# hliuson/ogbench

Measured on AMD Instinct MI355X. Metric: env steps/sec at N=65536 parallel envs, pointmaze-large, 1/2/4/8 MI355X, higher is better.
Workload: dtype f64; 1 GPU; pointmaze-large-navigate-v0; total_envs=65536, num_envs_per_gpu=65536, auto_reset=True, task_id=i%5+1, seed=0, parallelism=env-shard x1 (contiguous blocks, global env_base)

## Files before the change

ogbench_amd/csrc/locomaze.hip:

```cpp
#include <cmath>
#include <cstdlib>
#include <cstring>
#include <deque>
#include <string>
#include <type_traits>
#include <vector>

#include "common.h"
#include "goal_threshold.h"
#include "point_physics.h"
#include "point_contact.h"


namespace ogbx {

constexpr int kMaxCells = 256;
constexpr int kMaxTasks = 8;

struct MazeParams {
  PointModel pm;
  int32_t H, W, num_tasks, loco_type;
  int32_t success_pre, terminate_at_goal, add_noise_to_goal, reward_task_id;
  int32_t max_steps, n_tp_in, n_tp_out, pad_;
  int64_t env_base;
  double goal_tol, tp_radius;
  double tp_in[2][2];
  double tp_out[3][2];
  int32_t tasks[kMaxTasks][4];
  uint8_t wall[kMaxCells];
  uint16_t nbmask[kMaxCells];
};

struct MazeState {
  double* qpos;
  double* goal;
  int32_t* elapsed;
  int32_t* task;
  uint32_t* episode;
};

struct MazeStepConsts {
  const uint16_t* nbmask;
  int64_t env_base;
  double goal_tol;
  double goal_s2max;
  int32_t H, W, max_steps, n_tp_in;
  int32_t success_pre, terminate_at_goal, reward_task_id, add_noise_to_goal;
};

}

struct ogbx_maze_env {
  int32_t device = 0;
  int64_t n = 0;
  ogbx::MazeParams P;
  ogbx::MazeState S{};
  ogbx::MazeParams* Pd = nullptr;
  ogbx::MazeStepConsts C{};
  int16_t* bfs = nullptr;
  uint64_t seed = 0;
  bool was_reset = false;
  double* body_qpos = nullptr;
  double* body_qvel = nullptr;
  int epw = 64;
  int lds_pad = 0;
  bool bound = false;
  double* b_obs = nullptr;
  float* b_reward = nullptr;
  uint8_t *b_term = nullptr, *b_trunc = nullptr, *b_succ = nullptr;
  double* b_final = nullptr;
  int32_t b_auto = 0;
};

namespace ogbx {


#define OGBX_POINT_MODEL(pm, P) constexpr PointModel pm = kPointModel

__device__ inline void stage_wall(const MazeParams& P, uint8_t* wall_s) {
  for (int t = threadIdx.x; t < P.H * P.W; t += blockDim.x) wall_s[t] = P.wall[t];
  __syncthreads();
}

__device__ inline void stage_nbmask(const MazeParams& P, uint16_t* nb_s) {
  for (int t = threadIdx.x; t < P.H * P.W; t += blockDim.x) nb_s[t] = P.nbmask[t];
  __syncthreads();
}

static_assert(kMaxCells == kStepBlock, "one wall-mask entry per thread of a step block");

__device__ __forceinline__ uint16_t nbmask_fetch(const MazeParams* Pp) { return Pp->nbmask[threadIdx.x]; }

__device__ __forceinline__ void nbmask_commit(uint16_t* nb_s, uint16_t v) {
  nb_s[threadIdx.x] = v;
  __syncthreads();
}

__device__ inline bool goal_reached(double x, double y, double gx, double gy, double tol) {
  double dx = x - gx, dy = y - gy;
  return sqrt(fma(dy, dy, dx * dx)) <= tol;
}

__device__ inline bool goal_within(double x, double y, double gx, double gy, double s2max) {
  double dx = x - gx, dy = y - gy;
  return fma(dy, dy, dx * dx) <= s2max;
}

__device__ inline void reset_draws(uint64_t i, uint32_t ep, uint32_t k0, uint32_t k1,
                                   double r[4]) {
  u32x4 a = philox4x32_10({(uint32_t)i, ep, 0u, (uint32_t)(i >> 32)}, k0, k1);
  u32x4 b = philox4x32_10({(uint32_t)i, ep, 1u, (uint32_t)(i >> 32)}, k0, k1);
  r[0] = -1.0 + 2.0 * u01_from(a.x, a.y);
  r[1] = -1.0 + 2.0 * u01_from(a.z, a.w);
  r[2] = -1.0 + 2.0 * u01_from(b.x, b.y);
  r[3] = -1.0 + 2.0 * u01_from(b.z, b.w);
}

__device__ inline int32_t draw_task(const MazeParams& P, uint64_t i, uint32_t ep, uint32_t k0,
                                    uint32_t k1) {
  u32x4 c = philox4x32_10({(uint32_t)i, ep, 2u, (uint32_t)(i >> 32)}, k0, k1);
  return 1 + (int32_t)bounded_u32(c.x, (uint32_t)P.num_tasks);
}

__device__ inline void task_centres(const PointModel& pm, const int32_t* t, double c[4]) {
  c[0] = t[1] * pm.unit - pm.off_x;
  c[1] = t[0] * pm.unit - pm.off_y;
  c[2] = t[3] * pm.unit - pm.off_x;
  c[3] = t[2] * pm.unit - pm.off_y;
}

__device__ inline void reset_noise(const PointModel& pm, const double c[4], int32_t add_noise_to_goal,
                                   const double r[4], double& x, double& y, double& gx, double& gy) {
  x = c[0] + r[0] * pm.unit / 4.0;
  y = c[1] + r[1] * pm.unit / 4.0;
  if (add_noise_to_goal) {
    gx = c[2] + r[2] * pm.unit / 4.0;
    gy = c[3] + r[3] * pm.unit / 4.0;
  } else {
    gx = c[2];
    gy = c[3];
  }
}

__device__ inline void reset_one(const MazeParams& P, int32_t task, const double* task_xy,
                                 const double r[4], double& x, double& y, double& gx,
                                 double& gy) {
  double c[4];
  if (task_xy != nullptr) {
    for (int k = 0; k < 4; ++k) c[k] = task_xy[k];
  } else {
    task_centres(P.pm, P.tasks[task - 1], c);
  }
  reset_noise(P.pm, c, P.add_noise_to_goal, r, x, y, gx, gy);
}

__device__ inline void reset_from_task(const PointModel& pm, const int32_t* t, int32_t add_noise_to_goal,
                                       const double r[4], double& x, double& y, double& gx, double& gy) {
  double c[4];
  task_centres(pm, t, c);
  reset_noise(pm, c, add_noise_to_goal, r, x, y, gx, gy);
}


constexpr int kEpwReplicate = 0x100;

__device__ inline int64_t env_of_lane(int epw, bool* writer) {
  const int lane = threadIdx.x & 63;
  const int e = epw & 0xFF;
  const int64_t wave = ((int64_t)blockIdx.x * kStepBlock + threadIdx.x) >> 6;
  *writer = lane < e;
  if (lane >= e && !(epw & kEpwReplicate)) return -1;
  return wave * e + (lane & (e - 1));
}

__global__ void __launch_bounds__(256) maze_reset_kernel(const MazeParams* __restrict__ Pp, MazeState S, int64_t n,
                                                         const int32_t* task_id,
                                                         const double* task_xy,
                                                         const uint8_t* mask, const double* noise,
                                                         double* obs, double* goal_out,
                                                         uint32_t k0, uint32_t k1) {
  const MazeParams& P = *Pp;
  const PointModel pm = P.pm;
  int64_t i = (int64_t)blockIdx.x * blockDim.x + threadIdx.x;
  if (i >= n) return;
  if (mask != nullptr && mask[i] == 0) return;
  uint32_t ep = S.episode[i] + 1u;
  const uint64_t gi = (uint64_t)(i + P.env_base);
  int32_t task;
  if (P.reward_task_id > 0) task = P.reward_task_id;
  else if (task_id != nullptr) task = task_id[i];
  else task = draw_task(P, gi, ep, k0, k1);
  if (task < 1 || task > P.num_tasks) task = 1;
  double r[4];
  if (noise != nullptr) {
    r[0] = noise[4 * i + 0];
    r[1] = noise[4 * i + 1];
    r[2] = noise[4 * i + 2];
    r[3] = noise[4 * i + 3];
  } else {
    reset_draws(gi, ep, k0, k1, r);
  }
  double x, y, gx, gy;
  reset_one(P, task, task_xy ? task_xy + 4 * i : nullptr, r, x, y, gx, gy);
  S.qpos[2 * i] = x;
  S.qpos[2 * i + 1] = y;
  S.goal[2 * i] = gx;
  S.goal[2 * i + 1] = gy;
  S.elapsed[i] = 0;
  S.task[i] = task;
  S.episode[i] = ep;
  obs[2 * i] = x;
  obs[2 * i + 1] = y;
  goal_out[2 * i] = gx;
  goal_out[2 * i + 1] = gy;
}

#ifdef OGBX_WAVE_STAMPS
__device__ unsigned long long g_wave_stamps[4096 * 4];
#endif

typedef double f64x2 __attribute__((ext_vector_type(2)));

constexpr int64_t kPlainMaxEnvs = (int64_t)1 << 27;

template <bool k32, class T>
__device__ __forceinline__ T* env_elem(T* base, int64_t i) {
  if constexpr (k32) {
    using B = std::conditional_t<std::is_const_v<T>, const char, char>;
    return reinterpret_cast<T*>(reinterpret_cast<B*>(base) + (uint32_t)i * (uint32_t)sizeof(T));
  } else {
    return base + i;
  }
}

template <bool kF64, bool kUntilDone, bool kPlain = false>
__global__ void __launch_bounds__(256) maze_step_kernel(
    const MazeStepConsts C, MazeState S, const void* __restrict__ action_v, int64_t n,
    double* __restrict__ obs, float* __restrict__ reward, uint8_t* __restrict__ terminated,
    uint8_t* __restrict__ truncated, uint8_t* __restrict__ success, int32_t auto_reset, int32_t k_steps_arg,
    double* __restrict__ final_obs, uint32_t k0, uint32_t k1, int epw,
    const MazeParams* __restrict__ Pp, int32_t* __restrict__ steps_taken) {
  static_assert(!(kPlain && kUntilDone), "the plain instantiation is the single auto-reset step");
  const MazeParams& P = *Pp;
  OGBX_POINT_MODEL(pm, P);
  const int32_t k_steps = kPlain ? 1 : k_steps_arg;
  const int32_t n_tp_in = kPlain ? 0 : C.n_tp_in;
  __shared__ uint16_t nb_s[kMaxCells];
#ifdef OGBX_WAVE_STAMPS
  const unsigned long long ws_t0 = wall_clock64(), ws_c0 = clock64();
#endif
#ifdef OGBX_STAGE_STAMPS
  const unsigned long long ps_t0 = __builtin_amdgcn_s_memtime();
  __builtin_amdgcn_sched_barrier(0);
#endif
  bool writer = true;
  int64_t i;
  bool live;
  if constexpr (kPlain) {
    const uint32_t t = blockIdx.x * kStepBlock + threadIdx.x;
    i = t;
    live = t < (uint32_t)n;
  } else {
    i = env_of_lane(epw, &writer);
    live = i >= 0 && i < n;
  }
  asm volatile("" ::"s"(C.H), "s"(C.W), "s"(C.max_steps), "s"(C.goal_tol), "s"(action_v), "s"(S.episode),
               "s"(k_steps_arg));
  double2 q = make_double2(0.0, 0.0), g = q, a0d = q;
  float2 a0f = make_float2(0.0f, 0.0f);
  int32_t el = 0, task = 1;
  uint32_t ep = 0;
  if (live) {
    q = *env_elem<kPlain>(reinterpret_cast<const double2*>(S.qpos), i);
    if (kF64) a0d = *env_elem<kPlain>(reinterpret_cast<const double2*>(action_v), i);
    else a0f = *env_elem<kPlain>(reinterpret_cast<const float2*>(action_v), i);
    g = *env_elem<kPlain>(reinterpret_cast<const double2*>(S.goal), i);
    el = *env_elem<kPlain>(static_cast<const int32_t*>(S.elapsed), i);
  }
  const uint16_t nbv = C.nbmask[threadIdx.x];
#ifdef OGBX_STAGE_STAMPS
  asm volatile("s_waitcnt vmcnt(0)" ::: "memory");
  OGBX_PS_AT(1);
  path_stamp_store(0, ps_t0);
#endif
  nbmask_commit(nb_s, nbv);
  OGBX_PS_AT(2);
  if (!live) return;
  bool have_te = k_steps > 1 || n_tp_in > 0 || el + 1 >= C.max_steps;
  {
    const double ddx = q.x - g.x, ddy = q.y - g.y, lim = C.goal_tol + 2.0;
    have_te |= ddx * ddx + ddy * ddy <= lim * lim;
  }
  if (have_te) {
    ep = *env_elem<kPlain>(static_cast<const uint32_t*>(S.episode), i);
    task = *env_elem<kPlain>(static_cast<const int32_t*>(S.task), i);
  }
  const uint64_t gi = (uint64_t)(i + C.env_base);
  double x = q.x, y = q.y, gx = g.x, gy = g.y;
  bool reset_any = false;
  bool done = false;
  int32_t taken = 0;
  double dx_ = x, dy_ = y;
  int32_t del_ = el;

  for (int32_t k = 0; k < k_steps; ++k) {
    if (kUntilDone) {
      if (__all(done)) break;
    }
    const int64_t o = kPlain ? i : (int64_t)k * n + i;
    double dx, dy;
    if (kF64) {
      const double2 a = k == 0 ? a0d : reinterpret_cast<const double2*>(action_v)[o];
      dx = 0.2 * a.x;
      dy = 0.2 * a.y;
    } else {
      const float2 a = k == 0 ? a0f : reinterpret_cast<const float2*>(action_v)[o];
      dx = (double)(0.2f * a.x);
      dy = (double)(0.2f * a.y);
    }
    bool succ = false;
    if (C.success_pre) succ = goal_within(x, y, gx, gy, C.goal_s2max);
    x = x + dx;
    y = y + dy;
    if constexpr (kPlain) {
#pragma unroll 1
      for (int32_t rep = 0; rep < k_steps_arg; ++rep) point_step_as(pm, nb_s, C.H, C.W, &x, &y);
    } else {
      point_step_as(pm, nb_s, C.H, C.W, &x, &y);
    }
    if (!C.success_pre) succ = goal_within(x, y, gx, gy, C.goal_s2max);
    const double ox = x, oy = y;
    if (n_tp_in > 0) {
      for (int t = 0; t < n_tp_in; ++t) {
        if (goal_reached(x, y, P.tp_in[t][0], P.tp_in[t][1], P.tp_radius * 1.5)) {
          u32x4 c = philox4x32_10({(uint32_t)gi, ep, 0x100u + (uint32_t)el, (uint32_t)(gi >> 32)},
                                  k0 ^ kTagMazeTeleport, k1);
          int o_idx = (int)bounded_u32(c.x, (uint32_t)P.n_tp_out);
          x = P.tp_out[o_idx][0];
          y = P.tp_out[o_idx][1];
          break;
        }
      }
    }
    float rew = succ ? 1.0f : 0.0f;
    if (C.reward_task_id > 0) rew -= 1.0f;
    const bool term = succ && C.terminate_at_goal;
    el += 1;
    const bool trunc = el >= C.max_steps;
    const bool write = writer && (!kUntilDone || !done);
    if (write) {
      __builtin_nontemporal_store(rew, env_elem<kPlain>(reward, o));
      __builtin_nontemporal_store((uint8_t)term, env_elem<kPlain>(terminated, o));
      __builtin_nontemporal_store((uint8_t)trunc, env_elem<kPlain>(truncated, o));
      __builtin_nontemporal_store((uint8_t)succ, env_elem<kPlain>(success, o));
    }
    OGBX_PS_AT(8);
    double wx = ox, wy = oy;
    if (auto_reset && (term || trunc)) {
      if (!have_te) {
        ep = *env_elem<kPlain>(static_cast<const uint32_t*>(S.episode), i);
        task = *env_elem<kPlain>(static_cast<const int32_t*>(S.task), i);
        have_te = true;
      }
      if (final_obs != nullptr && writer)
        *env_elem<kPlain>(reinterpret_cast<double2*>(final_obs), o) = make_double2(ox, oy);
      ep += 1u;
      reset_any = true;
      double r[4];
      reset_draws(gi, ep, k0, k1, r);
      reset_from_task(pm, P.tasks[task - 1], C.add_noise_to_goal, r, x, y, gx, gy);
      el = 0;
      wx = x;
      wy = y;
    }
    if (write) __builtin_nontemporal_store(f64x2{wx, wy}, env_elem<kPlain>(reinterpret_cast<f64x2*>(obs), o));
    if (kUntilDone && !done) {
      taken = k + 1;
      done = term || trunc;
      dx_ = x;
      dy_ = y;
      del_ = el;
    }
  }
  if (kUntilDone) {
    x = dx_;
    y = dy_;
    el = del_;
    if (writer) steps_taken[i] = taken;
  }
  if (!writer) return;
  OGBX_PS_AT(9);
  __builtin_nontemporal_store(f64x2{x, y}, env_elem<kPlain>(reinterpret_cast<f64x2*>(S.qpos), i));
  __builtin_nontemporal_store(el, env_elem<kPlain>(S.elapsed, i));
  if (reset_any) {
    *env_elem<kPlain>(reinterpret_cast<double2*>(S.goal), i) = make_double2(gx, gy);
    *env_elem<kPlain>(S.episode, i) = ep;
  }
  OGBX_PS_AT(10);
#ifdef OGBX_WAVE_STAMPS
  {
    const unsigned long long t1 = wall_clock64(), c1 = clock64();
    const int64_t w = ((int64_t)blockIdx.x * kStepBlock + threadIdx.x) >> 6;
    if ((threadIdx.x & 63) == 0 && w < 4096) {
      g_wave_stamps[4 * w + 0] = ws_t0;
      g_wave_stamps[4 * w + 1] = t1;
      g_wave_stamps[4 * w + 2] = c1 - ws_c0;
    }
  }
#endif
}

template <bool kF64>
__global__ void __launch_bounds__(256) point_physics_kernel(const MazeParams* __restrict__ Pp,
                                                            const double* qpos_in,
                                                            const void* action_v, int64_t n,
                                                            double* qpos_out,
                                                            uint8_t* contact_out, int epw) {
  OGBX_POINT_MODEL(pm, (*Pp));
  __shared__ uint16_t nb_s[kMaxCells];
  bool writer;
  const int64_t i = env_of_lane(epw, &writer);
  const bool live = i >= 0 && i < n;
  const uint16_t nbv = nbmask_fetch(Pp);
  double x = 0.0, y = 0.0, ax = 0.0, ay = 0.0;
  if (live) {
    x = qpos_in[2 * i];
    y = qpos_in[2 * i + 1];
    if (kF64) {
      const double* a = (const double*)action_v;
      ax = 0.2 * a[2 * i];
      ay = 0.2 * a[2 * i + 1];
    } else {
      const float* a = (const float*)action_v;
      ax = (double)(0.2f * a[2 * i]);
      ay = (double)(0.2f * a[2 * i + 1]);
    }
  }
  nbmask_commit(nb_s, nbv);
  if (!live) return;
  const MazeParams& P = *Pp;
  x = x + ax;
  y = y + ay;
  int c = point_step_as(pm, nb_s, P.H, P.W, &x, &y);
  if (!writer) return;
  qpos_out[2 * i] = x;
  qpos_out[2 * i + 1] = y;
  if (contact_out) contact_out[i] = (uint8_t)c;
}

__global__ void xy_to_ij_kernel(const MazeParams* __restrict__ Pp, const double* xy, int64_t n, int32_t* ij) {
  const MazeParams& P = *Pp;
  const PointModel pm = P.pm;
  int64_t t = (int64_t)blockIdx.x * blockDim.x + threadIdx.x;
  if (t >= n) return;
  double x = xy[2 * t], y = xy[2 * t + 1];
  double fi = (y + P.pm.off_y + 0.5 * P.pm.unit) / P.pm.unit;
  double fj = (x + P.pm.off_x + 0.5 * P.pm.unit) / P.pm.unit;
  fi = fmin(fmax(fi, -2147483648.0), 2147483647.0);
  fj = fmin(fmax(fj, -2147483648.0), 2147483647.0);
  ij[2 * t] = (int32_t)fi;
  ij[2 * t + 1] = (int32_t)fj;
}

__global__ void ij_to_xy_kernel(const MazeParams* __restrict__ Pp, const int32_t* ij, int64_t n, double* xy) {
  const MazeParams& P = *Pp;
  const PointModel pm = P.pm;
  int64_t t = (int64_t)blockIdx.x * blockDim.x + threadIdx.x;
  if (t >= n) return;
  xy[2 * t] = ij[2 * t + 1] * P.pm.unit - P.pm.off_x;
  xy[2 * t + 1] = ij[2 * t] * P.pm.unit - P.pm.off_y;
}

__device__ inline int clamp_idx(double f, int hi) {
  f = fmin(fmax(f, -1.0), (double)hi);
  int v = (int)f;
  return v < 0 ? 0 : (v > hi - 1 ? hi - 1 : v);
}

__device__ inline void subgoal_of(const MazeParams& P, const uint8_t* wall_s, const int16_t* bfs, double x,
                                  double y, double gx, double gy, double* sx_out, double* sy_out) {
  const int H = P.H, W = P.W;
  const int si = clamp_idx((y + P.pm.off_y + 0.5 * P.pm.unit) / P.pm.unit, H);
  const int sj = clamp_idx((x + P.pm.off_x + 0.5 * P.pm.unit) / P.pm.unit, W);
  const int gi = clamp_idx((gy + P.pm.off_y + 0.5 * P.pm.unit) / P.pm.unit, H);
  const int gj = clamp_idx((gx + P.pm.off_x + 0.5 * P.pm.unit) / P.pm.unit, W);
  const int16_t* d = bfs + (int64_t)(gi * W + gj) * (H * W);
  int bi = si, bj = sj;
  const int di[4] = {-1, 0, 1, 0}, dj[4] = {0, -1, 0, 1};
#pragma unroll
  for (int k = 0; k < 4; ++k) {
    const int ni = si + di[k], nj = sj + dj[k];
    if (ni >= 0 && ni < H && nj >= 0 && nj < W && wall_s[ni * W + nj] == 0 && d[ni * W + nj] < d[bi * W + bj]) {
      bi = ni;
      bj = nj;
    }
  }
  *sx_out = bj * P.pm.unit - P.pm.off_x;
  *sy_out = bi * P.pm.unit - P.pm.off_y;
}

__global__ void oracle_subgoal_kernel(const MazeParams* __restrict__ Pp, const int16_t* bfs, const double* start_xy,
                                      const double* goal_xy, int64_t n, double* sub_xy) {
  const MazeParams& P = *Pp;
  __shared__ uint8_t wall_s[kMaxCells];
  stage_wall(P, wall_s);
  const int64_t t = (int64_t)blockIdx.x * blockDim.x + threadIdx.x;
  if (t >= n) return;
  subgoal_of(P, wall_s, bfs, start_xy[2 * t], start_xy[2 * t + 1], goal_xy[2 * t], goal_xy[2 * t + 1],
             &sub_xy[2 * t], &sub_xy[2 * t + 1]);
}

__global__ void expert_action_kernel(const MazeParams* __restrict__ Pp, const int16_t* bfs, const double* start_xy,
                                     const double* goal_xy, int64_t n, double noise, const double* normal,
                                     uint32_t k0, uint32_t k1, uint32_t call_lo, uint32_t call_hi,
                                     double* action) {
  const MazeParams& P = *Pp;
  __shared__ uint8_t wall_s[kMaxCells];
  stage_wall(P, wall_s);
  const int64_t t = (int64_t)blockIdx.x * blockDim.x + threadIdx.x;
  if (t >= n) return;
  const double x = start_xy[2 * t], y = start_xy[2 * t + 1];
  double sx, sy;
  subgoal_of(P, wall_s, bfs, x, y, goal_xy[2 * t], goal_xy[2 * t + 1], &sx, &sy);
  const double dx = sx - x, dy = sy - y;
  const double den = sqrt(fma(dy, dy, dx * dx)) + 1e-6;
  const double ux = dx / den, uy = dy / den;
  double nx, ny;
  if (normal != nullptr) {
    nx = normal[2 * t];
    ny = normal[2 * t + 1];
  } else {
    const uint64_t gt = (uint64_t)(t + P.env_base);
    const u32x4 w = philox4x32_10({(uint32_t)gt, call_lo, 0x45u, (uint32_t)(gt >> 32) ^ call_hi}, k0, k1);
    const double u1 = 1.0 - u01_from(w.x, w.y);
    const double u2 = u01_from(w.z, w.w);
    const double r = sqrt(-2.0 * log(u1));
    const double a = 6.283185307179586 * u2;
    nx = 0.0 + noise * (r * cos(a));
    ny = 0.0 + noise * (r * sin(a));
  }
  double ax = ux + nx, ay = uy + ny;
  ax = ax < -1.0 ? -1.0 : (ax > 1.0 ? 1.0 : ax);
  ay = ay < -1.0 ? -1.0 : (ay > 1.0 ? 1.0 : ay);
  action[2 * t] = ax;
  action[2 * t + 1] = ay;
}

__global__ void set_goal_kernel(const MazeParams* __restrict__ Pp, MazeState S, int64_t n, const int32_t* goal_ij,
                                const uint8_t* mask, const double* noise, uint32_t k0, uint32_t k1, uint32_t call_lo,
                                uint32_t call_hi) {
  const MazeParams& P = *Pp;
  const int64_t i = (int64_t)blockIdx.x * blockDim.x + threadIdx.x;
  if (i >= n || (mask != nullptr && mask[i] == 0)) return;
  double gx = goal_ij[2 * i + 1] * P.pm.unit - P.pm.off_x;
  double gy = goal_ij[2 * i] * P.pm.unit - P.pm.off_y;
  if (P.add_noise_to_goal) {
    double r0, r1;
    if (noise != nullptr) {
      r0 = noise[2 * i];
      r1 = noise[2 * i + 1];
    } else {
      const uint64_t gi = (uint64_t)(i + P.env_base);
      const u32x4 w = philox4x32_10({(uint32_t)gi, call_lo, 0x47u, (uint32_t)(gi >> 32) ^ call_hi}, k0, k1);
      r0 = -1.0 + 2.0 * u01_from(w.x, w.y);
      r1 = -1.0 + 2.0 * u01_from(w.z, w.w);
    }
    gx = gx + r0 * P.pm.unit / 4.0;
    gy = gy + r1 * P.pm.unit / 4.0;
  }
  reinterpret_cast<double2*>(S.goal)[i] = make_double2(gx, gy);
}

}

#include "antmaze.h"

namespace ogbx {


struct MazeSpec {
  const char* name;
  int H, W;
  const char* rows;
  int ntasks;
  int tasks[5][4];
};

static const MazeSpec kMazes[] = {
    {"arena", 8, 8,
     "11111111"
     "10000001"
     "10000001"
     "10000001"
     "10000001"
     "10000001"
     "10000001"
     "11111111",
     1, {{1, 1, 6, 6}}},
    {"medium", 8, 8,
     "11111111"
     "10011001"
     "10010001"
     "11000111"
     "10010001"
     "10100101"
     "10001001"
     "11111111",
     5, {{1, 1, 6, 6}, {6, 1, 1, 6}, {5, 3, 4, 2}, {6, 5, 6, 1}, {2, 6, 1, 1}}},
    {"large", 9, 12,
     "111111111111"
     "100001000001"
     "101101010101"
     "100000010001"
     "101111011101"
     "100101000001"
     "110101010111"
     "100100010001"
     "111111111111",
     5, {{1, 1, 7, 10}, {5, 4, 7, 1}, {7, 4, 1, 10}, {3, 8, 5, 4}, {1, 1, 5, 4}}},
    {"giant", 12, 16,
     "1111111111111111"
     "1010000001100001"
     "1010110101001101"
     "1000100100010001"
     "1011101111110101"
     "1000100010000101"
     "1110101001010111"
     "1000100100010001"
     "1010101111110101"
     "1011100010001101"
     "1000001000100001"
     "1111111111111111",
     5, {{1, 1, 10, 14}, {1, 14, 10, 1}, {8, 14, 1, 1}, {8, 3, 5, 12}, {5, 9, 3, 8}}},
    {"teleport", 9, 12,
     "111111111111"
     "100000101001"
     "110100010011"
     "110111000001"
     "100001010101"
     "101101010101"
     "101101010101"
     "100001000101"
     "111111111111",
     5, {{1, 10, 7, 1}, {1, 1, 7, 10}, {5, 6, 7, 10}, {7, 1, 7, 10}, {5, 6, 7, 1}}},
};


static void build_bfs(const MazeParams& P, std::vector<int16_t>& out) {
  const int H = P.H, W = P.W, C = H * W;
  out.assign((size_t)C * C, -1);
  for (int g = 0; g < C; ++g) {
    int16_t* d = out.data() + (size_t)g * C;
    std::deque<int> qu;
    d[g] = 0;
    qu.push_back(g);
    const int di[4] = {-1, 0, 1, 0}, dj[4] = {0, -1, 0, 1};
    while (!qu.empty()) {
      int c = qu.front();
      qu.pop_front();
      int i = c / W, j = c % W;
      for (int k = 0; k < 4; ++k) {
        int ni = i + di[k], nj = j + dj[k];
        if (ni >= 0 && ni < H && nj >= 0 && nj < W && P.wall[ni * W + nj] == 0 &&
            d[ni * W + nj] == -1) {
          d[ni * W + nj] = (int16_t)(d[c] + 1);
          qu.push_back(ni * W + nj);
        }
      }
    }
  }
}

static inline uint32_t grid_for(int64_t n, int block) { return (uint32_t)((n + block - 1) / block); }

}

using namespace ogbx;

extern "C" {

ogbx_status ogbx_maze_create(const char* maze_type, int64_t n_envs, int32_t device,
                             const ogbx_maze_opts* opts, ogbx_maze_t* out) {
  OGBX_CHECK(out != nullptr && maze_type != nullptr && opts != nullptr, OGBX_EINVAL,
             "ogbx_maze_create: null argument");
  *out = nullptr;
  OGBX_CHECK(n_envs > 0 && n_envs <= (int64_t)1 << 32, OGBX_EINVAL,
             "ogbx_maze_create: n_envs must be in [1, 2^32]");
  const MazeSpec* spec = nullptr;
  for (const auto& s : kMazes)
    if (std::strcmp(s.name, maze_type) == 0) spec = &s;
  OGBX_CHECK(spec != nullptr, OGBX_EINVAL, std::string("Unknown maze type: ") + maze_type);
  OGBX_CHECK(opts->loco_type >= 0 && opts->loco_type <= 2, OGBX_EINVAL,
             "Unknown locomotion environment type");
  OGBX_CHECK(opts->success_timing == 0 || opts->success_timing == 1, OGBX_EINVAL,
             "success_timing must be 'pre' or 'post'");
  OGBX_CHECK(opts->max_episode_steps > 0, OGBX_EINVAL, "max_episode_steps must be positive");
  OGBX_CHECK(opts->env_base >= 0, OGBX_EINVAL, "env_base must be >= 0");
  OGBX_CHECK(opts->reward_task_id <= spec->ntasks, OGBX_EINVAL,
             "Task ID must be in [1, " + std::to_string(spec->ntasks) + "].");
// ... 497 lines not shown
```

Measured before the change: 5.921 billion env_steps/s.

## Use per-wave nbmask tables and defer kernarg loads in plain step kernel

In the plain single-step instantiation, each wave now stages its own copy of the neighbour-mask table in LDS using 8-byte pieces and a wave barrier, replacing the block-wide __syncthreads. Tail lanes are clamped to a valid env instead of returning early, so every lane takes part in the staging. Epilogue scalars and pointers are reloaded from the kernarg segment after the physics loop rather than held in SGPRs throughout, which is meant to reduce register pressure. The cost is more LDS per block and extra scalar loads, and the code relies on a hand-mirrored kernarg layout guarded by static_asserts.

New measurement: 6.203 billion env_steps/s, median of 6. 4.8% higher.

```diff
diff --git a/ogbench_amd/csrc/locomaze.hip b/ogbench_amd/csrc/locomaze.hip
--- a/ogbench_amd/csrc/locomaze.hip
+++ b/ogbench_amd/csrc/locomaze.hip
@@ -1,4 +1,5 @@
 #include <cmath>
+#include <cstddef>
 #include <cstdlib>
 #include <cstring>
 #include <deque>
@@ -46,6 +47,40 @@
   double goal_s2max;
   int32_t H, W, max_steps, n_tp_in;
   int32_t success_pre, terminate_at_goal, reward_task_id, add_noise_to_goal;
+};
+
+struct MazeStepArgs {
+  MazeStepConsts C;
+  MazeState S;
+  const void* action;
+  int64_t n;
+  double* obs;
+  float* reward;
+  uint8_t *terminated, *truncated, *success;
+  int32_t auto_reset, k_steps;
+  double* final_obs;
+  uint32_t k0, k1;
+  int32_t epw;
+  const MazeParams* Pp;
+  int32_t* steps_taken;
+};
+static_assert(offsetof(MazeStepArgs, S) == 0x40 && offsetof(MazeStepArgs, n) == 0x70 &&
+                  offsetof(MazeStepArgs, obs) == 0x78 && offsetof(MazeStepArgs, final_obs) == 0xa8 &&
+                  offsetof(MazeStepArgs, Pp) == 0xc0 && sizeof(MazeStepArgs) == 0xd0,
+              "MazeStepArgs mirrors maze_step_kernel's kernarg layout");
+
+struct MazeStepTail {
+  int64_t n, env_base;
+  double goal_s2max;
+  int32_t max_steps, success_pre, terminate_at_goal, reward_task_id, add_noise_to_goal, auto_reset;
+  uint32_t k0, k1;
+  const MazeParams* Pp;
+  double *obs, *final_obs;
+  float* reward;
+  uint8_t *terminated, *truncated, *success;
+  double *qpos, *goal;
+  int32_t* elapsed;
+  uint32_t* episode;
 };
 
 }
@@ -95,6 +130,10 @@
   nb_s[threadIdx.x] = v;
   __syncthreads();
 }
+
+typedef uint64_t u64_alias __attribute__((may_alias));
+static_assert(kMaxCells * sizeof(uint16_t) == 64 * sizeof(uint64_t), "one 8-byte piece of the table per lane of a wave");
+static_assert(offsetof(MazeParams, nbmask) % sizeof(uint64_t) == 0, "the table is read in 8-byte pieces");
 
 __device__ inline bool goal_reached(double x, double y, double gx, double gy, double tol) {
   double dx = x - gx, dy = y - gy;
@@ -233,6 +272,34 @@
   }
 }
 
+template <class ArgsPtr>
+__device__ __forceinline__ MazeStepTail step_tail(ArgsPtr a) {
+  MazeStepTail T;
+  T.n = a->n;
+  T.env_base = a->C.env_base;
+  T.goal_s2max = a->C.goal_s2max;
+  T.max_steps = a->C.max_steps;
+  T.success_pre = a->C.success_pre;
+  T.terminate_at_goal = a->C.terminate_at_goal;
+  T.reward_task_id = a->C.reward_task_id;
+  T.add_noise_to_goal = a->C.add_noise_to_goal;
+  T.auto_reset = a->auto_reset;
+  T.k0 = a->k0;
+  T.k1 = a->k1;
+  T.Pp = a->Pp;
+  T.obs = a->obs;
+  T.final_obs = a->final_obs;
+  T.reward = a->reward;
+  T.terminated = a->terminated;
+  T.truncated = a->truncated;
+  T.success = a->success;
+  T.qpos = a->S.qpos;
+  T.goal = a->S.goal;
+  T.elapsed = a->S.elapsed;
+  T.episode = a->S.episode;
+  return T;
+}
+
 template <bool kF64, bool kUntilDone, bool kPlain = false>
 __global__ void __launch_bounds__(256) maze_step_kernel(
     const MazeStepConsts C, MazeState S, const void* __restrict__ action_v, int64_t n,
@@ -245,7 +312,8 @@
   OGBX_POINT_MODEL(pm, P);
   const int32_t k_steps = kPlain ? 1 : k_steps_arg;
   const int32_t n_tp_in = kPlain ? 0 : C.n_tp_in;
-  __shared__ uint16_t nb_s[kMaxCells];
+  __shared__ __attribute__((aligned(8))) uint16_t nb_s[kPlain ? kStepBlock / 64 * kMaxCells : kMaxCells];
+  const uint16_t* nb = nb_s;
 #ifdef OGBX_WAVE_STAMPS
   const unsigned long long ws_t0 = wall_clock64(), ws_c0 = clock64();
 #endif
@@ -257,15 +325,22 @@
   int64_t i;
   bool live;
   if constexpr (kPlain) {
+    asm volatile("" ::"s"(n), "s"(C.nbmask), "s"(C.H), "s"(C.W), "s"(C.success_pre), "s"(C.goal_s2max), "s"(action_v),
+                 "s"(S.qpos), "s"(S.goal), "s"(S.elapsed), "s"(S.task), "s"(S.episode), "s"(k_steps_arg));
+  } else {
+    asm volatile("" ::"s"(C.H), "s"(C.W), "s"(C.max_steps), "s"(C.goal_tol), "s"(action_v), "s"(S.episode),
+                 "s"(k_steps_arg));
+  }
+  if constexpr (kPlain) {
     const uint32_t t = blockIdx.x * kStepBlock + threadIdx.x;
-    i = t;
-    live = t < (uint32_t)n;
+    if ((uint32_t)__builtin_amdgcn_readfirstlane((int)t) >= (uint32_t)n) return;
+    live = true;
+    writer = t < (uint32_t)n;
+    i = writer ? t : (uint32_t)n - 1u;
   } else {
     i = env_of_lane(epw, &writer);
     live = i >= 0 && i < n;
   }
-  asm volatile("" ::"s"(C.H), "s"(C.W), "s"(C.max_steps), "s"(C.goal_tol), "s"(action_v), "s"(S.episode),
-               "s"(k_steps_arg));
   double2 q = make_double2(0.0, 0.0), g = q, a0d = q;
   float2 a0f = make_float2(0.0f, 0.0f);
   int32_t el = 0, task = 1;
@@ -277,25 +352,49 @@
     g = *env_elem<kPlain>(reinterpret_cast<const double2*>(S.goal), i);
     el = *env_elem<kPlain>(static_cast<const int32_t*>(S.elapsed), i);
   }
-  const uint16_t nbv = C.nbmask[threadIdx.x];
-#ifdef OGBX_STAGE_STAMPS
-  asm volatile("s_waitcnt vmcnt(0)" ::: "memory");
-  OGBX_PS_AT(1);
-  path_stamp_store(0, ps_t0);
-#endif
-  nbmask_commit(nb_s, nbv);
-  OGBX_PS_AT(2);
-  if (!live) return;
-  bool have_te = k_steps > 1 || n_tp_in > 0 || el + 1 >= C.max_steps;
-  {
-    const double ddx = q.x - g.x, ddy = q.y - g.y, lim = C.goal_tol + 2.0;
-    have_te |= ddx * ddx + ddy * ddy <= lim * lim;
-  }
-  if (have_te) {
+  bool have_te;
+  if constexpr (kPlain) {
     ep = *env_elem<kPlain>(static_cast<const uint32_t*>(S.episode), i);
     task = *env_elem<kPlain>(static_cast<const int32_t*>(S.task), i);
-  }
-  const uint64_t gi = (uint64_t)(i + C.env_base);
+    have_te = true;
+    const uint64_t nbv = reinterpret_cast<const u64_alias*>(C.nbmask)[threadIdx.x & 63];
+#ifdef OGBX_STAGE_STAMPS
+    asm volatile("s_waitcnt vmcnt(0)" ::: "memory");
+    OGBX_PS_AT(1);
+    path_stamp_store(0, ps_t0);
+#endif
+    reinterpret_cast<u64_alias*>(nb_s)[threadIdx.x] = nbv;
+    __builtin_amdgcn_fence(__ATOMIC_RELEASE, "wavefront");
+    __builtin_amdgcn_wave_barrier();
+    __builtin_amdgcn_fence(__ATOMIC_ACQUIRE, "wavefront");
+    nb = nb_s + (threadIdx.x >> 6) * kMaxCells;
+    OGBX_PS_AT(2);
+  } else {
+    const uint16_t nbv = C.nbmask[threadIdx.x];
+#ifdef OGBX_STAGE_STAMPS
+    asm volatile("s_waitcnt vmcnt(0)" ::: "memory");
+    OGBX_PS_AT(1);
+    path_stamp_store(0, ps_t0);
+#endif
+    nbmask_commit(nb_s, nbv);
+    OGBX_PS_AT(2);
+    if (!live) return;
+    have_te = k_steps > 1 || n_tp_in > 0 || el + 1 >= C.max_steps;
+    {
+      const double ddx = q.x - g.x, ddy = q.y - g.y, lim = C.goal_tol + 2.0;
+      have_te |= ddx * ddx + ddy * ddy <= lim * lim;
+    }
+    if (have_te) {
+      ep = *env_elem<kPlain>(static_cast<const uint32_t*>(S.episode), i);
+      task = *env_elem<kPlain>(static_cast<const int32_t*>(S.task), i);
+    }
+  }
+  MazeStepTail T;
+  if constexpr (!kPlain) {
+    const MazeStepArgs A{C,  S,  action_v, n,   obs, reward, terminated, truncated,  success, auto_reset, k_steps_arg,
+                         final_obs, k0, k1, epw, Pp,  steps_taken};
+    T = step_tail(&A);
+  }
   double x = q.x, y = q.y, gx = g.x, gy = g.y;
   bool reset_any = false;
   bool done = false;
@@ -323,12 +422,26 @@
     x = x + dx;
     y = y + dy;
     if constexpr (kPlain) {
+      int32_t rep = 0;
 #pragma unroll 1
-      for (int32_t rep = 0; rep < k_steps_arg; ++rep) point_step_as(pm, nb_s, C.H, C.W, &x, &y);
+      do point_step_as(pm, nb, C.H, C.W, &x, &y);
+      while (++rep < k_steps_arg);
     } else {
-      point_step_as(pm, nb_s, C.H, C.W, &x, &y);
-    }
-    if (!C.success_pre) succ = goal_within(x, y, gx, gy, C.goal_s2max);
+      point_step_as(pm, nb, C.H, C.W, &x, &y);
+    }
+    if constexpr (kPlain) {
+      auto A = (const __attribute__((address_space(4))) MazeStepArgs*)__builtin_amdgcn_kernarg_segment_ptr();
+      asm volatile("" : "+s"(A));
+      T = step_tail(A);
+      asm volatile("" ::"s"(T.n), "s"(T.env_base), "s"(T.goal_s2max), "s"(T.max_steps), "s"(T.success_pre),
+                   "s"(T.terminate_at_goal), "s"(T.reward_task_id), "s"(T.add_noise_to_goal), "s"(T.auto_reset),
+                   "s"(T.k0), "s"(T.k1), "s"(T.Pp));
+      asm volatile("" ::"s"(T.obs), "s"(T.final_obs), "s"(T.reward), "s"(T.terminated), "s"(T.truncated),
+                   "s"(T.success), "s"(T.qpos), "s"(T.goal), "s"(T.elapsed), "s"(T.episode));
+      writer = (uint32_t)(blockIdx.x * kStepBlock + threadIdx.x) < (uint32_t)T.n;
+    }
+    const uint64_t gi = (uint64_t)(i + T.env_base);
+    if (!T.success_pre) succ = goal_within(x, y, gx, gy, T.goal_s2max);
     const double ox = x, oy = y;
     if (n_tp_in > 0) {
       for (int t = 0; t < n_tp_in; ++t) {
@@ -343,37 +456,37 @@
       }
     }
     float rew = succ ? 1.0f : 0.0f;
-    if (C.reward_task_id > 0) rew -= 1.0f;
-    const bool term = succ && C.terminate_at_goal;
+    if (T.reward_task_id > 0) rew -= 1.0f;
+    const bool term = succ && T.terminate_at_goal;
     el += 1;
-    const bool trunc = el >= C.max_steps;
+    const bool trunc = el >= T.max_steps;
     const bool write = writer && (!kUntilDone || !done);
     if (write) {
-      __builtin_nontemporal_store(rew, env_elem<kPlain>(reward, o));
-      __builtin_nontemporal_store((uint8_t)term, env_elem<kPlain>(terminated, o));
-      __builtin_nontemporal_store((uint8_t)trunc, env_elem<kPlain>(truncated, o));
-      __builtin_nontemporal_store((uint8_t)succ, env_elem<kPlain>(success, o));
+      __builtin_nontemporal_store(rew, env_elem<kPlain>(T.reward, o));
+      __builtin_nontemporal_store((uint8_t)term, env_elem<kPlain>(T.terminated, o));
+      __builtin_nontemporal_store((uint8_t)trunc, env_elem<kPlain>(T.truncated, o));
+      __builtin_nontemporal_store((uint8_t)succ, env_elem<kPlain>(T.success, o));
     }
     OGBX_PS_AT(8);
     double wx = ox, wy = oy;
-    if (auto_reset && (term || trunc)) {
+    if (T.auto_reset && (term || trunc)) {
       if (!have_te) {
-        ep = *env_elem<kPlain>(static_cast<const uint32_t*>(S.episode), i);
+        ep = *env_elem<kPlain>(static_cast<const uint32_t*>(T.episode), i);
         task = *env_elem<kPlain>(static_cast<const int32_t*>(S.task), i);
         have_te = true;
       }
-      if (final_obs != nullptr && writer)
-        *env_elem<kPlain>(reinterpret_cast<double2*>(final_obs), o) = make_double2(ox, oy);
+      if (T.final_obs != nullptr && writer)
+        *env_elem<kPlain>(reinterpret_cast<double2*>(T.final_obs), o) = make_double2(ox, oy);
       ep += 1u;
       reset_any = true;
       double r[4];
-      reset_draws(gi, ep, k0, k1, r);
-      reset_from_task(pm, P.tasks[task - 1], C.add_noise_to_goal, r, x, y, gx, gy);
+      reset_draws(gi, ep, T.k0, T.k1, r);
+      reset_from_task(pm, T.Pp->tasks[task - 1], T.add_noise_to_goal, r, x, y, gx, gy);
       el = 0;
       wx = x;
       wy = y;
     }
-    if (write) __builtin_nontemporal_store(f64x2{wx, wy}, env_elem<kPlain>(reinterpret_cast<f64x2*>(obs), o));
+    if (write) __builtin_nontemporal_store(f64x2{wx, wy}, env_elem<kPlain>(reinterpret_cast<f64x2*>(T.obs), o));
     if (kUntilDone && !done) {
       taken = k + 1;
       done = term || trunc;
@@ -390,11 +503,11 @@
   }
   if (!writer) return;
   OGBX_PS_AT(9);
-  __builtin_nontemporal_store(f64x2{x, y}, env_elem<kPlain>(reinterpret_cast<f64x2*>(S.qpos), i));
-  __builtin_nontemporal_store(el, env_elem<kPlain>(S.elapsed, i));
+  __builtin_nontemporal_store(f64x2{x, y}, env_elem<kPlain>(reinterpret_cast<f64x2*>(T.qpos), i));
+  __builtin_nontemporal_store(el, env_elem<kPlain>(T.elapsed, i));
   if (reset_any) {
-    *env_elem<kPlain>(reinterpret_cast<double2*>(S.goal), i) = make_double2(gx, gy);
-    *env_elem<kPlain>(S.episode, i) = ep;
+    *env_elem<kPlain>(reinterpret_cast<double2*>(T.goal), i) = make_double2(gx, gy);
+    *env_elem<kPlain>(T.episode, i) = ep;
   }
   OGBX_PS_AT(10);
 #ifdef OGBX_WAVE_STAMPS
```
